# antonilo/unsupervised_detection

Measured on AMD Instinct MI355X. Metric: frame-pairs/sec per adversarial step, DAVIS 480p batch4, 1/2/4/8 GPU, higher is better.
Workload: dtype f32

## Files before the change

### include/udet_debug.h

```cpp
#ifndef UDET_DEBUG_H
#define UDET_DEBUG_H
#include <stddef.h>
#ifdef __cplusplus
extern "C" {
#endif
void udet_debug_force_conv(int bm, int bn, int ks);
void udet_debug_conv_fp16(int on);
void udet_debug_conv_fp16_grad_scale(float s);
void udet_debug_force_wgrad(int nsplit, int dma);
int udet_debug_last_wgrad(void);
int udet_debug_last_wgrad_reduce(void);
int udet_debug_conv2d_backward_filter_ex(const float* x, int ldx, int x_coff, const float* dy, int ldy, int y_coff, const float* y_saved, int act,
                                         float alpha, const float* w, const float* b, const float* gamma, float bn_c, float* dw, float* db,
                                         float* dgamma, float* dbeta, int n, int h, int wd, int cin, int cout, int k, int stride, int dilation,
                                         int up, void* workspace, size_t workspace_bytes, void* stream);
void udet_debug_upb_min_pixels(long v);
void udet_debug_set_tuning(int on);
void udet_debug_force_pair(int on);
int udet_debug_last_pair(void);
int udet_debug_conv2d_pair(const float* xa, const float* xb, const float* wa, const float* wb, const float* ba, const float* bb, float* ya, float* yb,
                           int na, int nb, int h, int w, int cin, int cout, int k, int stride, int dilation, int act, float alpha, void* workspace,
                           size_t workspace_bytes, void* stream);
#define UDET_DEBUG_UPCONV_WSETS_OFFSET 6400
size_t udet_debug_upconv_lowres_workspace_bytes(int ldx, int cin, int cout);
int udet_debug_upconv_lowres_fwd(const float* x, int ldx, const float* w, const float* bias, int act, float alpha, float* y, int ldy, int y_coff,
                                 float* xhat, int n, int h, int wd, int cin, int cout, int split, void* workspace, size_t workspace_bytes,
                                 void* stream);
int udet_debug_upconv_lowres_bwd(const float* dy, int ldy, int y_coff, const float* w, float* dx, int ldx, float* dxhat, int n, int h, int wd,
                                 int cin, int cout, void* workspace, size_t workspace_bytes, void* stream);
int udet_debug_upconv_tables(int h, int w, int backward, int* nseg, int* seg, int* seg_tap, int* taps, int taps_cap, int* ntaps);
int udet_debug_max_segs(void);
int udet_debug_last_conv(void);
#ifdef __cplusplus
}
#endif
#endif
```

### unsupervised_detection_amd/_devel.py

```python
from __future__ import annotations

import ctypes
import os

from ._ffi import check as _check, lib as _lib

_PATH = os.path.join(os.path.dirname(os.path.abspath(__file__)), "libudet_debug.so")
if not os.path.exists(_PATH):
    raise RuntimeError(f"{_PATH} is missing: build it with `make -C unsupervised_detection_amd/csrc`")
dbg = ctypes.CDLL(_PATH, mode=ctypes.RTLD_GLOBAL)
dbg.udet_debug_force_conv.restype = None
dbg.udet_debug_force_conv.argtypes = [ctypes.c_int, ctypes.c_int, ctypes.c_int]
dbg.udet_debug_last_conv.restype = ctypes.c_int
dbg.udet_debug_last_conv.argtypes = []
dbg.udet_debug_conv_fp16.restype = None
dbg.udet_debug_conv_fp16.argtypes = [ctypes.c_int]
dbg.udet_debug_conv_fp16_grad_scale.restype = None
dbg.udet_debug_conv_fp16_grad_scale.argtypes = [ctypes.c_float]
dbg.udet_debug_force_wgrad.restype = None
dbg.udet_debug_force_wgrad.argtypes = [ctypes.c_int, ctypes.c_int]
dbg.udet_debug_upb_min_pixels.restype = None
dbg.udet_debug_upb_min_pixels.argtypes = [ctypes.c_long]
dbg.udet_debug_set_tuning.restype = None
dbg.udet_debug_set_tuning.argtypes = [ctypes.c_int]
dbg.udet_debug_last_wgrad.restype = ctypes.c_int
dbg.udet_debug_last_wgrad.argtypes = []
dbg.udet_debug_force_pair.restype = None
dbg.udet_debug_force_pair.argtypes = [ctypes.c_int]
dbg.udet_debug_last_pair.restype = ctypes.c_int
dbg.udet_debug_last_pair.argtypes = []
dbg.udet_debug_conv2d_pair.restype = ctypes.c_int
dbg.udet_debug_conv2d_pair.argtypes = [ctypes.c_void_p] * 8 + [ctypes.c_int] * 10 + [ctypes.c_float, ctypes.c_void_p, ctypes.c_size_t, ctypes.c_void_p]
dbg.udet_debug_last_wgrad_reduce.restype = ctypes.c_int
dbg.udet_debug_last_wgrad_reduce.argtypes = []
_p, _i, _f = ctypes.c_void_p, ctypes.c_int, ctypes.c_float
dbg.udet_debug_conv2d_backward_filter_ex.restype = ctypes.c_int
dbg.udet_debug_conv2d_backward_filter_ex.argtypes = ([_p, _i, _i, _p, _i, _i, _p, _i, _f, _p, _p, _p, _f, _p, _p, _p, _p] + [_i] * 9
                                                     + [_p, ctypes.c_size_t, _p])
UPCONV_WSETS_OFFSET = 6400
dbg.udet_debug_upconv_lowres_workspace_bytes.restype = ctypes.c_size_t
dbg.udet_debug_upconv_lowres_workspace_bytes.argtypes = [_i, _i, _i]
dbg.udet_debug_upconv_lowres_fwd.restype = ctypes.c_int
dbg.udet_debug_upconv_lowres_fwd.argtypes = [_p, _i, _p, _p, _i, _f, _p, _i, _i, _p] + [_i] * 6 + [_p, ctypes.c_size_t, _p]
dbg.udet_debug_upconv_lowres_bwd.restype = ctypes.c_int
dbg.udet_debug_upconv_lowres_bwd.argtypes = [_p, _i, _i, _p, _p, _i, _p] + [_i] * 5 + [_p, ctypes.c_size_t, _p]
dbg.udet_debug_upconv_tables.restype = ctypes.c_int
dbg.udet_debug_upconv_tables.argtypes = [_i, _i, _i] + [_p] * 4 + [_i, _p]
dbg.udet_debug_max_segs.restype = ctypes.c_int
dbg.udet_debug_max_segs.argtypes = []


def upconv_tables(h: int, w: int, backward: bool):
    cap = 1024
    nseg, ntaps = ctypes.c_int(0), ctypes.c_int(0)
    seg, seg_tap, taps = (ctypes.c_int * 64)(), (ctypes.c_int * 17)(), (ctypes.c_int * (3 * cap))()
    st = dbg.udet_debug_upconv_tables(h, w, 1 if backward else 0, ctypes.addressof(nseg), ctypes.addressof(seg), ctypes.addressof(seg_tap),
                                      ctypes.addressof(taps), cap, ctypes.addressof(ntaps))
    _check(st)
    ns, nt = nseg.value, ntaps.value
    return dict(nseg=ns, seg=[tuple(seg[4 * s:4 * s + 4]) for s in range(ns)], seg_tap=list(seg_tap[:ns + 1]),
                taps=[tuple(taps[3 * t:3 * t + 3]) for t in range(nt)])
```

### unsupervised_detection_amd/csrc/conv_host.h

```cpp
#pragma once
#include "common.h"
namespace udet {
void same_pad(int in, int k, int s, int d, int* before, int* out);
void conv_setup_fwd(ConvParams& p, int N, int H, int W, int kh, int kw, int s, int d);
int conv_dgrad_classes(int s, int H, int W);
void conv_force_config(int bm, int bn, int ks);
bool conv_thin_n_ok(const ConvParams& p);
bool conv_thin_k_ok(const ConvParams& p);
int launch_conv_thin_n(const ConvParams& p, hipStream_t stream);
int launch_conv_thin_k(const ConvParams& p, hipStream_t stream);
bool conv_wino_geometry(const ConvParams& p, int* dil, int widx_at[9]);
bool conv_wino_ok(const ConvParams& p);
bool conv_wino_variant_ok(const ConvParams& p, int variant);
int conv_wino_np(int cout);
size_t conv_wino_floats(int Kc, int cout);
long conv_wino_workgroups(const ConvParams& p, int variant);
int conv_wino_max_ksplit(const ConvParams& p, int variant);
int launch_conv_wino(ConvParams& p, int variant, int ks, hipStream_t stream);
int launch_splitk_second_pass(const ConvParams& p, hipStream_t stream);
int launch_wino_pack(const float* src, float* dst, int R, int C, int Kc, int np, int k_split, int k_gap, int transposed, hipStream_t stream);
int launch_wino_from_packed(const ConvParams& p, float* dst, int np, hipStream_t stream);
void conv_debug_f16(int on);
int conv_debug_f16_on();
void conv_debug_f16_grad_scale(float s);
float conv_debug_f16_grad_scale_now();
int conv_last_config();
void conv_set_tuning(int on);
int tuned_shapes();
void tune_dump(FILE* f);
bool tune_put_line(const char* line);
int conv_tune_rejected();
void wgrad_set_tuning(int on);
bool wgrad_wino_ok(const WgradParams& p);
int wgrad_wino_slices(const WgradParams& p, int wanted);
int launch_wgrad_wino(const WgradParams& q, int slices, int ldn, hipStream_t stream);
int wgrad_last_config();
enum { WGRAD_RED_FUSED_BN = 1 << 26, WGRAD_RED_SEPARATE_BN = 1 << 27, WGRAD_RED_SWAPPED = 1 << 28, WGRAD_RED_CLASSES = 1 << 29 };
int wgrad_last_reduce();
void setup_up_fwd(ConvParams& p, int N, int H, int W);
void wgrad_force(int nsplit, int dma);
void conv_force_pair(int on);
int conv_last_pair();
#define UDET_TUNE_ABI 6
bool conv_setup_dgrad(ConvParams& p, int cls, int N, int H, int W, int kh, int kw, int s, int d);
int launch_pack_weights(const float* src, float* dst, int T, int R, int C, int Kc, int ldw, int k_split, int k_gap,
                        int mode, const float* scale, hipStream_t stream);
int launch_pack_taps_into_n(const float* src, float* dst, int T, int R, int C, int Kc, int ldz, int k_split, int k_gap,
                            int transposed, hipStream_t stream);
int launch_pack_jobs(const PackJob* jobs_dev, int njobs, const float* wsrc, float* ws, float bn_c, hipStream_t stream);
int launch_fold_bn(const float* b, const float* gamma, const float* beta, float c, float* scale, float* bias_f, int n,
                   hipStream_t stream);
int launch_copy_channels(const float* src, int lds, int s_coff, float* dst, int ldd, int d_coff, long P, int C, float mul,
                         float add, hipStream_t stream);
int launch_warp(const float* img, const float* flow, int ldf, int f_coff, float flow_scale, float* out, int N, int H,
                int W, int C, int* dbg_idx, float* dbg_alpha, hipStream_t stream);
int launch_cost_volume(const float* c1, const float* wr, float* out, int ldo, int o_coff, int N, int H, int W, int C,
                       hipStream_t stream);
int launch_warp_cost_volume(const float* c1, const float* c2, const float* flow, int ldf, int f_coff, float flow_scale, float* out,
                            int ldo, int corr_coff, int c1_coff, float* warped_dbg, int N, int H, int W, int C, hipStream_t stream);
inline int round_up(int v, int m) { return (v + m - 1) / m * m; }
}
```

### unsupervised_detection_amd/csrc/conv_wino.hip

```cpp
#include <string.h>

#include <mutex>
#include <type_traits>

#include "common.h"
#include "conv_epilogue.h"
#include "conv_host.h"
#include "wino_pack.h"

namespace udet {

typedef float floatx16 __attribute__((ext_vector_type(16)));

#ifdef UDET_EXPERIMENT
__device__ long long g_wino_ts[512 * 8];
#define WINO_STAMP(i)                                                                                  \
  do {                                                                                                 \
    if (threadIdx.x == 0 && blockIdx.x < 512 && blockIdx.z == 0) g_wino_ts[blockIdx.x * 8 + (i)] = (long long)__builtin_readcyclecounter(); \
  } while (0)
extern "C" int udet_exp_wino_stamps(long long* host, int n) {
  return (int)hipMemcpyFromSymbol(host, HIP_SYMBOL(g_wino_ts), (size_t)(n < 512 * 8 ? n : 512 * 8) * sizeof(long long));
}
#else
#define WINO_STAMP(i) do {} while (0)
#endif

static constexpr int wino_row_slots(int pw) { return (pw + 3) / 8 * 8 + 4; }

template <int WTY, int WTX, int WN>
struct WinoGeom {
  static constexpr int NS = 3;
  static constexpr int TH = 4 * WTY, TW = 8 * WTX;
  static constexpr int PH = 2 * TH + 2, PW = 2 * TW + 2;
  static constexpr int CS = PW / 2;
  static constexpr int S = wino_row_slots(PW);
  static constexpr int HP = S / 2;
  static constexpr int IN_SLOTS = 2 * PH * S;
  static constexpr int IN_INSTR = (IN_SLOTS + 255) / 256;
  static constexpr int IN_BYTES = IN_INSTR * 256 * 16;
  static constexpr int BN = 32 * WN;
  static constexpr int W_BYTES = 16 * 2 * BN * 16;
  static constexpr int W_INSTR = W_BYTES / 4096;
  static constexpr int STAGE = IN_BYTES + W_BYTES;
  static constexpr int L = IN_INSTR + W_INSTR;
  static constexpr int LA = (L + 1) / 2;
  static constexpr int LDS_BYTES = NS * STAGE;
  static_assert(S % 8 == 4 && S >= PW && HP >= CS, "row stride");
  static_assert(LDS_BYTES >= 4 * 128 * 32 * 4 && LDS_BYTES <= 160 * 1024, "the epilogue transposes 16 KB per wave through the stage buffers");
};

__device__ __forceinline__ float4 wino_bias_prefetch(const ConvParams& p, int n4) {
  return (p.ksplit <= 1 && (p.Cout & 3) == 0 && n4 < p.Cout) ? epi4_bias(p, n4) : make_float4(0.f, 0.f, 0.f, 0.f);
}
__device__ __forceinline__ void wino_store_block(const ConvParams& p, const float* xp, int lane, int n4, int n, int d, int sy, int sx, int Hs, int Ws,
                                                 int Yb, int Xb, const float4& bias_pre) {
  const bool slab = p.ksplit > 1;
  const bool vec = slab ? ((reinterpret_cast<uintptr_t>(p.partial) & 15) == 0 && (p.ldp & 3) == 0) : epilogue4_out_ok(p);
  const int c4 = (lane & 7) * 4;
  if (!slab && vec) {
    if (n4 >= p.Cout) return;
    const float4 bias = bias_pre;
    const EpiAct ea = epi_act(p);
    auto pix = [&](int P) {
      const int m = P >> 2, a = (P >> 1) & 1, b = P & 1;
      const int oy = Yb + 2 * (m >> 3) + a, ox = Xb + 2 * (m & 7) + b;
      return (oy >= Hs || ox >= Ws) ? -1 : (n * p.H + sy + d * oy) * p.W + sx + d * ox;
    };
    auto loop = [&](auto ELU) {
      if (epi4_plain(p)) {
#pragma unroll 1
        for (int k0 = 0; k0 < 16; k0 += 4) {
          float4 v[4];
          int off[4];
#pragma unroll
          for (int u = 0; u < 4; ++u) {
            const int P = (k0 + u) * 8 + (lane >> 3);
            v[u] = *reinterpret_cast<const float4*>(&xp[P * 32 + c4]);
            off[u] = pix(P);
          }
#pragma unroll
          for (int u = 0; u < 4; ++u)
            if (off[u] >= 0) epi4_finish_plain32<decltype(ELU)::value>(p, off[u], n4, v[u], bias, ea.slope);
        }
        return;
      }
#pragma unroll 1
      for (int k0 = 0; k0 < 16; k0 += 8) {
        float4 v[8];
        int off[8];
        Epi4Req rq[8];
#pragma unroll
        for (int u = 0; u < 8; ++u) {
          const int P = (k0 + u) * 8 + (lane >> 3);
          v[u] = *reinterpret_cast<const float4*>(&xp[P * 32 + c4]);
          off[u] = pix(P);
          if (off[u] >= 0) epi4_request(p, off[u], n4, rq[u]);
        }
#pragma unroll
        for (int u = 0; u < 8; ++u)
          if (off[u] >= 0) epi4_finish<decltype(ELU)::value>(p, off[u], n4, v[u], bias, rq[u], ea);
      }
    };
    if (p.act == ACT_ELU) loop(std::true_type());
// ... 290 lines not shown
      constexpr int RA[4] = {0, 1, 2, 1}, RB[4] = {2, 2, 1, 3};
      float vv[4][4];
#pragma unroll
      for (int j = 0; j < 4; ++j) {
        float t[4];
#pragma unroll
        for (int c = 0; c < 4; ++c) {
          const float a = comp(row[RA[i]][c], j), b = comp(row[RB[i]][c], j);
          t[c] = i == 1 ? a + b : a - b;
        }
        vv[j][0] = t[0] - t[2];
        vv[j][1] = t[1] + t[2];
        vv[j][2] = t[2] - t[1];
        vv[j][3] = t[1] - t[3];
      }
      __builtin_amdgcn_sched_barrier(0);
#pragma unroll
      for (int j = 0; j < 4; ++j)
#pragma unroll
        for (int q = 0; q < 4; ++q)
          acc[4 * i + q] = __builtin_amdgcn_mfma_f32_32x32x2f32(vv[j][q], comp(bfr[i & 1][q], j), acc[4 * i + q], 0, 0, 0);
      __builtin_amdgcn_sched_barrier(0);
      if (i == 2) {
        asm volatile("s_waitcnt vmcnt(0)" ::: "memory");
        __builtin_amdgcn_s_barrier();
        asm volatile("" ::: "memory");
      }
    }
    buf = b1;
  }

  __syncthreads();
  float* xp = reinterpret_cast<float*>(smem) + wave * (128 * 32);
#pragma unroll
  for (int r = 0; r < 16; ++r) {
    const int m = (r & 3) + 8 * (r >> 2) + 4 * lh;
    float s[4][2];
#pragma unroll
    for (int i = 0; i < 4; ++i) {
      s[i][0] = acc[i * 4 + 0][r] + acc[i * 4 + 1][r] + acc[i * 4 + 2][r];
      s[i][1] = acc[i * 4 + 1][r] - acc[i * 4 + 2][r] - acc[i * 4 + 3][r];
    }
#pragma unroll
    for (int b = 0; b < 2; ++b) {
      xp[(m * 4 + b) * 32 + li] = s[0][b] + s[1][b] + s[2][b];
      xp[(m * 4 + 2 + b) * 32 + li] = s[1][b] - s[2][b] - s[3][b];
    }
  }
  __builtin_amdgcn_wave_barrier();
  wino_store_block(p, xp, lane, nb * BN + wn * 32 + (lane & 7) * 4, n, d, sy, sx, Hs, Ws, Y0 + 8 * wty, X0 + 16 * wtx, bias_pre);
}

template <int WTY, int WTX, int WN>
__global__ __launch_bounds__(512) __attribute__((amdgpu_waves_per_eu(2, 2))) void conv_wino8_kernel(const ConvParams p, const int dil,
                                                                                                   const int BY, const int BX) {
  static_assert(WTY * WTX * WN == 4, "4 wave tiles");
  typedef WinoGeom<WTY, WTX, WN> G;
  constexpr int NS = G::NS, TH = G::TH, TW = G::TW, PH = G::PH, S = G::S, HP = G::HP, CS = G::CS;
  constexpr int IN_INSTR = G::IN_INSTR, IN_BYTES = G::IN_BYTES, BN = G::BN, STAGE = G::STAGE;
  constexpr int NW = G::W_BYTES / 1024;
  constexpr int PER = (IN_INSTR * 4 + NW + 7) / 8;
  constexpr int W0 = PER > IN_INSTR ? PER - IN_INSTR : 0;
  constexpr int W1 = (NW - 4 * W0) / 4;
  static_assert(W1 >= 0 && 4 * W0 + 4 * W1 == NW, "weight split");
  extern __shared__ __attribute__((aligned(16))) char smem[];
  WINO_STAMP(0);

  const int tid = threadIdx.x, lane = tid & 63, wave = __builtin_amdgcn_readfirstlane(tid >> 6);
  const int role = wave >> 2, sub = wave & 3;
  const int li = lane & 31, lh = lane >> 5;
  const int wn = sub % WN, wt = sub / WN, wty = wt / WTX, wtx = wt % WTX;

  int bid = xcd_tile_order(blockIdx.x, gridDim.x);
  const int NB = (p.Cout + BN - 1) / BN;
  const int nb = bid % NB;
  bid /= NB;
  const int d = dil;
  const int bx = bid % BX;
  int rem = bid / BX;
  const int by = rem % BY;
  rem /= BY;
  const int sx = rem % d;
  rem /= d;
  const int sy = rem % d;
  const int n = rem / d;
  const int Hs = (p.H - sy + d - 1) / d, Ws = (p.W - sx + d - 1) / d;
  const int Y0 = by * 2 * TH, X0 = bx * 2 * TW;
  const int nkg_all = p.Kc >> 3;
  int kg0 = 0, kg1 = nkg_all;
  if (p.ksplit > 1) {
    kg0 = (int)((long)nkg_all * blockIdx.z / p.ksplit);
    kg1 = (int)((long)nkg_all * (blockIdx.z + 1) / p.ksplit);
  }
  const int nkg = kg1 - kg0;

  unsigned in_voff[IN_INSTR];
  unsigned long long in_mask[IN_INSTR];
#pragma unroll
  for (int i = 0; i < IN_INSTR; ++i) {
    const int Lx = (i * 4 + sub) * 64 + lane;
    const int quad = Lx / (PH * S), r2 = Lx - quad * (PH * S);
    const int row = r2 / S, s = r2 - row * S;
    const int par = s / HP, cs = s - par * HP;
    const int col = 2 * cs + par;
    const int yy = Y0 - 1 + row, xx = X0 - 1 + col;
    const bool ok = quad < 2 && cs < CS && yy >= 0 && yy < Hs && xx >= 0 && xx < Ws;
    in_voff[i] = ok ? (unsigned)(((n * p.H + sy + d * yy) * p.W + sx + d * xx) * p.ldx + p.x_coff + quad * 4) * 4u : 0u;
    in_mask[i] = __ballot(ok);
    if (!ok && role == 0) {
#pragma unroll
      for (int b = 0; b < NS; ++b) *reinterpret_cast<float4*>(smem + b * STAGE + Lx * 16) = make_float4(0.f, 0.f, 0.f, 0.f);
    }
  }
  __syncthreads();
  WINO_STAMP(1);
  const int np = p.wino_np;
  const float4 bias_pre = wino_bias_prefetch(p, nb * BN + wn * 32 + (lane & 7) * 4);
  const float* ubase = p.wino_u + (size_t)nb * BN * 4;
  const size_t ustride = (size_t)32 * np * 4;
  const unsigned w_voff = BN == 32 ? (unsigned)((lane >> 5) * np + (lane & 31)) * 16 : (unsigned)lane * 16;
  const unsigned lds0 = (unsigned)(uintptr_t)(__attribute__((address_space(3))) char*)smem;
  auto dma_in = [&](int kg, int buf, int i) {
    asm volatile("s_mov_b32 m0, %2\n\ts_mov_b64 exec, %3\n\tglobal_load_lds_dwordx4 %0, %1\n\ts_mov_b64 exec, -1" ::"v"(in_voff[i]), "s"(p.x + kg * 8),
                 "s"(lds0 + buf * STAGE + (i * 4 + sub) * 1024), "s"(in_mask[i])
                 : "m0");
  };
  auto dma_w = [&](int kg, int buf, int w) {
    const float* us = ubase + (size_t)kg * ustride + (BN == 64 ? (size_t)w * np * 4 : (size_t)(2 * w) * np * 4);
    asm volatile("s_mov_b32 m0, %2\n\tglobal_load_lds_dwordx4 %0, %1" ::"v"(w_voff), "s"(us), "s"(lds0 + buf * STAGE + IN_BYTES + w * 1024) : "m0");
  };
  auto dma_part = [&](auto ROLE, int kg, int buf, int i0, int i1) {
    constexpr int R = decltype(ROLE)::value;
    constexpr int LR = R == 0 ? IN_INSTR + W0 : W1;
#pragma unroll
    for (int i = 0; i < LR; ++i) {
      if (i < i0 || i >= i1) continue;
      if (R == 0) {
        if (i < IN_INSTR) dma_in(kg, buf, i);
        else dma_w(kg, buf, (i - IN_INSTR) * 4 + sub);
      } else {
        dma_w(kg, buf, 4 * W0 + i * 4 + sub);
      }
    }
  };

  floatx16 acc[8];
#pragma unroll
  for (int q = 0; q < 8; ++q)
#pragma unroll
    for (int r = 0; r < 16; ++r) acc[q][r] = 0.f;

  const int ty = li >> 3, tx = li & 7;
  const int a_base = ((lh * PH + 2 * (wty * 4 + ty)) * S + (wtx * 8 + tx)) * 16;
  const int b_base = IN_BYTES + (lh * BN + wn * 32 + li) * 16;
  auto ld_row = [&](const char* sb, int r, float4 (&dst)[4]) {
#pragma unroll
    for (int c = 0; c < 4; ++c) dst[c] = *reinterpret_cast<const float4*>(sb + a_base + (r * S + (c & 1) * HP + (c >> 1)) * 16);
  };
  auto ld_bf = [&](const char* sb, int i, float4 (&dst)[4]) {
#pragma unroll
    for (int q = 0; q < 4; ++q) dst[q] = *reinterpret_cast<const float4*>(sb + b_base + (4 * i + q) * (2 * BN * 16));
  };
  auto comp = [](const float4& v, int j) { return j == 0 ? v.x : (j == 1 ? v.y : (j == 2 ? v.z : v.w)); };

  auto body = [&](auto ROLE) {
    constexpr int R = decltype(ROLE)::value;
    constexpr int LR = R == 0 ? IN_INSTR + W0 : W1;
    constexpr int LA = (LR + 1) / 2;
    constexpr int I0 = R == 0 ? 1 : 0, I1 = R == 0 ? 2 : 3;
    float4 ra[4], rb[4];
    float4 rc[4], rd[4];
    float4 bf0[4], bf1[4];
    float v1[4][4];
#pragma unroll
    for (int c = 0; c < 4; ++c) ra[c] = rb[c] = rc[c] = rd[c] = bf0[c] = bf1[c] = make_float4(0.f, 0.f, 0.f, 0.f);
    if (nkg > 0) dma_part(ROLE, kg0, 0, 0, LR);
    if (nkg > 1) dma_part(ROLE, kg0 + 1, 1, 0, LR);
    if (nkg > 1) asm volatile("s_waitcnt vmcnt(%0)" ::"n"(LR) : "memory");
    else asm volatile("s_waitcnt vmcnt(0)" ::: "memory");
    __builtin_amdgcn_s_barrier();
    asm volatile("" ::: "memory");
    WINO_STAMP(2);
    ld_row(smem, R == 0 ? 1 : 0, ra);
    ld_row(smem, 2, rb);
    ld_bf(smem, I0, bf0);
    int buf = 0;
    for (int k = 0; k < nkg; ++k) {
      const char* sb = smem + buf * STAGE;
      const int b1 = buf + 1 == NS ? 0 : buf + 1, b2 = b1 + 1 == NS ? 0 : b1 + 1;
      const char* sbn = smem + b1 * STAGE;
      if (R == 1) { ld_row(sb, 1, rc); ld_row(sb, 3, rd); }
      ld_bf(sb, I1, bf1);
      if (k > 0 && k + 1 < nkg) dma_part(ROLE, kg0 + k + 1, b1, LA, LR);
      __builtin_amdgcn_sched_barrier(0);
#pragma unroll
      for (int j = 0; j < 4; ++j) {
        float t[4], v[4];
#pragma unroll
        for (int c = 0; c < 4; ++c) {
          const float a = comp(ra[c], j), b = comp(rb[c], j);
          t[c] = R == 0 ? a + b : a - b;
        }
        v[0] = t[0] - t[2]; v[1] = t[1] + t[2]; v[2] = t[2] - t[1]; v[3] = t[1] - t[3];
        if (R == 0) {
          float u[4];
#pragma unroll
          for (int c = 0; c < 4; ++c) u[c] = comp(rb[c], j) - comp(ra[c], j);
          v1[j][0] = u[0] - u[2]; v1[j][1] = u[1] + u[2]; v1[j][2] = u[2] - u[1]; v1[j][3] = u[1] - u[3];
        }
#pragma unroll
        for (int q = 0; q < 4; ++q) acc[q] = __builtin_amdgcn_mfma_f32_32x32x2f32(v[q], comp(bf0[q], j), acc[q], 0, 0, 0);
      }
      __builtin_amdgcn_sched_barrier(0);
      asm volatile("s_waitcnt vmcnt(0)" ::: "memory");
      __builtin_amdgcn_s_barrier();
      asm volatile("" ::: "memory");
      ld_row(sbn, R == 0 ? 1 : 0, ra);
      ld_row(sbn, 2, rb);
      ld_bf(sbn, I0, bf0);
      if (k + 2 < nkg) dma_part(ROLE, kg0 + k + 2, b2, 0, LA);
      __builtin_amdgcn_sched_barrier(0);
#pragma unroll
      for (int j = 0; j < 4; ++j) {
        float v[4];
        if (R == 0) {
#pragma unroll
          for (int q = 0; q < 4; ++q) v[q] = v1[j][q];
        } else {
          float t[4];
#pragma unroll
          for (int c = 0; c < 4; ++c) t[c] = comp(rc[c], j) - comp(rd[c], j);
          v[0] = t[0] - t[2]; v[1] = t[1] + t[2]; v[2] = t[2] - t[1]; v[3] = t[1] - t[3];
        }
#pragma unroll
        for (int q = 0; q < 4; ++q) acc[4 + q] = __builtin_amdgcn_mfma_f32_32x32x2f32(v[q], comp(bf1[q], j), acc[4 + q], 0, 0, 0);
      }
      __builtin_amdgcn_sched_barrier(0);
      buf = b1;
    }
  };
  if (role == 0) body(std::integral_constant<int, 0>());
  else body(std::integral_constant<int, 1>());

  WINO_STAMP(3);
  __syncthreads();
  wino_roles_epilogue(p, acc, reinterpret_cast<float*>(smem) + sub * 4096, role, lane, nb * BN + wn * 32 + (lane & 7) * 4, n, d, sy, sx, Hs, Ws, Y0 + 8 * wty,
                      X0 + 16 * wtx, bias_pre);
#ifdef UDET_EXPERIMENT
  WINO_STAMP(5);
  asm volatile("s_waitcnt vmcnt(0)" ::: "memory");
  WINO_STAMP(6);
#endif
}

struct WinoHalfGeom {
  static constexpr int NS = 2, TH = 4, TW = 8;
  static constexpr int PH = 2 * TH + 2, PW = 2 * TW + 2;
  static constexpr int CS = PW / 2, S = wino_row_slots(PW), HP = S / 2;
  static constexpr int IN_SLOTS = 2 * PH * S;
  static constexpr int IN_WINSTR = (IN_SLOTS + 63) / 64;
  static constexpr int IN_INSTR = (IN_WINSTR + 3) / 4;
  static constexpr int IN_BYTES = IN_WINSTR * 1024;
  static constexpr int BN = 64;
  static constexpr int W_BYTES = 16 * 2 * BN * 16;
  static constexpr int NW = W_BYTES / 1024;
  static constexpr int STAGE = IN_BYTES + W_BYTES;
  static constexpr int LDS_BYTES = NS * STAGE;
  static_assert(LDS_BYTES >= 4 * 128 * 32 * 4 && 2 * LDS_BYTES <= 160 * 1024, "epilogue scratch / two workgroups per CU");
};
__global__ __launch_bounds__(256) __attribute__((amdgpu_waves_per_eu(2, 2))) void conv_wino_half_kernel(const ConvParams p, const int dil, const int BY,
                                                                                                       const int BX) {
  typedef WinoHalfGeom G;
  constexpr int TH = G::TH, TW = G::TW, PH = G::PH, S = G::S, HP = G::HP, CS = G::CS;
  constexpr int IN_INSTR = G::IN_INSTR, IN_BYTES = G::IN_BYTES, BN = G::BN, STAGE = G::STAGE, NW = G::NW;
  extern __shared__ __attribute__((aligned(16))) char smem[];

  const int tid = threadIdx.x, lane = tid & 63, wave = __builtin_amdgcn_readfirstlane(tid >> 6);
  const int role = wave >> 1, wn = wave & 1;
  const int li = lane & 31, lh = lane >> 5;

  int bid = xcd_tile_order(blockIdx.x, gridDim.x);
  const int NB = (p.Cout + BN - 1) / BN;
  const int nb = bid % NB;
  bid /= NB;
  const int d = dil;
  const int bx = bid % BX;
  int rem = bid / BX;
  const int by = rem % BY;
  rem /= BY;
  const int sx = rem % d;
  rem /= d;
  const int sy = rem % d;
  const int n = rem / d;
  const int Hs = (p.H - sy + d - 1) / d, Ws = (p.W - sx + d - 1) / d;
  const int Y0 = by * 2 * TH, X0 = bx * 2 * TW;
  const int nkg_all = p.Kc >> 3;
  int kg0 = 0, kg1 = nkg_all;
  if (p.ksplit > 1) {
// ... 162 lines not shown
      for (int a = 0; a < 3; ++a)
#pragma unroll
        for (int b = 0; b < 3; ++b) val += Gm[pi][a] * Gm[pj][b] * wp[((long)tm.w[a * 3 + b] * Kc + k) * ldw + n];
    }
    dst[e] = val;
  }
}
int launch_wino_from_packed(const ConvParams& p, float* dst, int np, hipStream_t stream) {
  int d = 0;
  WinoTapMap tm;
  if (!conv_wino_geometry(p, &d, tm.w)) {
    set_error("wino: the launch is not a 3x3 stride-1 convolution");
    return UDET_ERR_UNSUPPORTED;
  }
  const long total = (long)(p.Kc / 8) * 16 * 2 * np * 4;
  int nb = (int)((total + 255) / 256);
  if (nb > 2048) nb = 2048;
  UDET_LAUNCH(wino_from_packed_kernel, dim3(nb), dim3(256), 0, stream, p.wp, p.Kc, p.ldw, tm, dst, np, total);
  UDET_HIP(hipGetLastError());
  return UDET_OK;
}

int conv_wino_np(int cout) { return cout > 64 ? round_up(cout, 128) : (cout > 32 ? 64 : 32); }
size_t conv_wino_floats(int Kc, int cout) { return (size_t)(Kc / 8) * 16 * 2 * conv_wino_np(cout) * 4; }

bool conv_wino_geometry(const ConvParams& p, int* dil, int widx_at[9]) {
  if (p.ntaps != 9 || p.ncls == 4 || p.up_shift != 0) return false;
  if (p.isy != 1 || p.isx != 1 || p.osy != 1 || p.osx != 1 || p.ooy != 0 || p.oox != 0) return false;
  if (p.OH != p.H || p.OW != p.W || p.OHq != p.OH || p.OWq != p.OW) return false;
  int d = 0;
  for (int t = 0; t < 9; ++t) {
    const int a = p.taps[t].dy < 0 ? -p.taps[t].dy : p.taps[t].dy;
    if (a > d) d = a;
  }
  if (d < 1) return false;
  for (int i = 0; i < 9; ++i) widx_at[i] = -1;
  for (int t = 0; t < 9; ++t) {
    const int dy = p.taps[t].dy, dx = p.taps[t].dx;
    if (dy % d != 0 || dx % d != 0) return false;
    const int a = dy / d + 1, b = dx / d + 1;
    if (a < 0 || a > 2 || b < 0 || b > 2 || widx_at[a * 3 + b] >= 0) return false;
    widx_at[a * 3 + b] = p.taps[t].widx;
  }
  *dil = d;
  return true;
}
bool conv_wino_ok(const ConvParams& p) {
  if (p.nseg) return false;
  int d, w[9];
  if (p.f16 || p.xa != nullptr || p.wino_u == nullptr || p.zero16 == nullptr) return false;
  if ((reinterpret_cast<uintptr_t>(p.zero16) | reinterpret_cast<uintptr_t>(p.wino_u) | reinterpret_cast<uintptr_t>(p.x)) & 15) return false;
  if (p.Kc < 8 || p.Kc % 8 != 0 || p.ldx % 4 != 0 || p.x_coff % 4 != 0) return false;
  if (p.wino_np < 32 || p.wino_np % 32 != 0 || p.wino_np < p.Cout) return false;
  if ((long)p.N * p.H * p.W * (long)p.ldy >= (1L << 31) || (long)p.N * p.H * p.W * (long)p.ldx >= (1L << 30)) return false;
  return conv_wino_geometry(p, &d, w);
}
static int variant_bn(int v) { return v == 4 ? 64 : ((v & 1) == 0 ? 64 : 32); }
bool conv_wino_variant_ok(const ConvParams& p, int v) {
  if (v < 0 || v > 4) return false;
  const int bn = variant_bn(v);
  if (p.wino_np % bn != 0) return false;
  return p.Cout > bn / 2 || bn == 32;
}
static void variant_blocks(const ConvParams& p, int v, int d, int* BY, int* BX) {
  const int th = v == 4 ? 4 : 8, tw = (v & 1) ? 16 : 8;
  const int Hs = (p.H + d - 1) / d, Ws = (p.W + d - 1) / d;
  *BY = (Hs + 2 * th - 1) / (2 * th);
  *BX = (Ws + 2 * tw - 1) / (2 * tw);
}
long conv_wino_workgroups(const ConvParams& p, int v) {
  int d, w[9], BY, BX;
  if (!conv_wino_geometry(p, &d, w)) return 0;
  variant_blocks(p, v, d, &BY, &BX);
  return (long)p.N * d * d * BY * BX * ((p.Cout + variant_bn(v) - 1) / variant_bn(v));
}
int conv_wino_max_ksplit(const ConvParams& p, int v) {
  (void)v;
  if (!p.partial) return 1;
  int ks = (p.Kc / 8) / 6;
  if (ks > 16) ks = 16;
  const size_t per_split = (size_t)p.N * p.H * p.W * ((p.Cout + 3) & ~3);
  while (ks > 1 && per_split * ks > p.partial_cap) --ks;
  return ks < 1 ? 1 : ks;
}
int launch_splitk_second_pass(const ConvParams& p, hipStream_t stream);

template <int WTY, int WTX, int WN, bool EIGHT>
static int launch_variant(const ConvParams& p, int d, int BY, int BX, hipStream_t stream) {
  typedef WinoGeom<WTY, WTX, WN> G;
  auto kern = EIGHT ? conv_wino8_kernel<WTY, WTX, WN> : conv_wino_kernel<WTY, WTX, WN>;
  static std::once_flag once;
  static hipError_t attr = hipSuccess;
  std::call_once(once, [&]() { attr = hipFuncSetAttribute(reinterpret_cast<const void*>(kern), hipFuncAttributeMaxDynamicSharedMemorySize, G::LDS_BYTES); });
  UDET_HIP(attr);
  dim3 grid(p.N * d * d * BY * BX * ((p.Cout + G::BN - 1) / G::BN), 1, p.ksplit > 1 ? p.ksplit : 1);
  UDET_LAUNCH(kern, grid, dim3(EIGHT ? 512 : 256), G::LDS_BYTES, stream, p, d, BY, BX);
  UDET_HIP(hipGetLastError());
  return UDET_OK;
}
static int launch_half(const ConvParams& p, int d, int BY, int BX, hipStream_t stream) {
  typedef WinoHalfGeom G;
  static std::once_flag once;
  static hipError_t attr = hipSuccess;
  std::call_once(once, [&]() { attr = hipFuncSetAttribute(reinterpret_cast<const void*>(conv_wino_half_kernel), hipFuncAttributeMaxDynamicSharedMemorySize, G::LDS_BYTES); });
  UDET_HIP(attr);
  dim3 grid(p.N * d * d * BY * BX * ((p.Cout + G::BN - 1) / G::BN), 1, p.ksplit > 1 ? p.ksplit : 1);
  UDET_LAUNCH(conv_wino_half_kernel, grid, dim3(256), G::LDS_BYTES, stream, p, d, BY, BX);
  UDET_HIP(hipGetLastError());
  return UDET_OK;
}
int launch_conv_wino(ConvParams& p, int variant, int ks, hipStream_t stream) {
  int d, w[9], BY, BX;
  if (!conv_wino_ok(p) || !conv_wino_geometry(p, &d, w) || !conv_wino_variant_ok(p, variant)) {
    set_error("wino: launch not eligible (variant %d)", variant);
    return UDET_ERR_UNSUPPORTED;
  }
  variant_blocks(p, variant, d, &BY, &BX);
  const int cap = conv_wino_max_ksplit(p, variant);
  p.ksplit = ks > cap ? cap : (ks < 1 ? 1 : ks);
  p.fold = 0; p.tail_full = 0; p.tail_ks = 0; p.tail_prow0 = 0;
  p.ncls = 1;
  if (p.ksplit > 1) p.ldp = (p.Cout + 3) & ~3;
  int rc;
  if (variant == 0) rc = launch_variant<2, 1, 2, false>(p, d, BY, BX, stream);
  else if (variant == 1) rc = launch_variant<2, 2, 1, false>(p, d, BY, BX, stream);
  else if (variant == 2) rc = launch_variant<2, 1, 2, true>(p, d, BY, BX, stream);
  else if (variant == 4) rc = launch_half(p, d, BY, BX, stream);
  else rc = launch_variant<2, 2, 1, true>(p, d, BY, BX, stream);
  if (rc != UDET_OK) return rc;
  if (p.ksplit > 1) return launch_splitk_second_pass(p, stream);
  return UDET_OK;
}

}
```

### unsupervised_detection_amd/csrc/devel/api_debug.hip

```cpp
#include <string.h>

#include <vector>

#include "../../../include/udet_debug.h"
#include "../conv_host.h"
#include "../plan_run.h"

using namespace udet;

extern "C" {
int udet_debug_last_conv(void) { return conv_last_config(); }
void udet_debug_force_conv(int bm, int bn, int ks) { conv_force_config(bm, bn, ks); }
void udet_debug_conv_fp16(int on) { conv_debug_f16(on); }
void udet_debug_conv_fp16_grad_scale(float s) { conv_debug_f16_grad_scale(s); }
void udet_debug_force_wgrad(int nsplit, int dma) { wgrad_force(nsplit, dma); }
int udet_debug_last_wgrad(void) { return wgrad_last_config(); }
int udet_debug_last_wgrad_reduce(void) { return wgrad_last_reduce(); }
int udet_debug_conv2d_backward_filter_ex(const float* x, int ldx, int x_coff, const float* dy, int ldy, int y_coff, const float* y_saved, int act,
                                         float alpha, const float* w, const float* b, const float* gamma, float bn_c, float* dw, float* db,
                                         float* dgamma, float* dbeta, int n, int h, int wd, int cin, int cout, int k, int stride, int dilation,
                                         int up, void* workspace, size_t workspace_bytes, void* stream_) {
  hipStream_t stream = (hipStream_t)stream_;
  if (!x || !dy || !dw || n < 1 || h < 1 || wd < 1 || cin < 1 || cout < 1 || k < 1 || k * k > UDET_MAX_TAPS || dilation < 1 ||
      (stride != 1 && stride != 2) || up < 0 || up > 2) {
    set_error("debug_backward_filter_ex: bad argument");
    return UDET_ERR_ARG;
  }
  if (ldx % 4 || x_coff % 4 || ldy % 4 || y_coff % 4) {
    set_error("debug_backward_filter_ex: ldx=%d x_coff=%d ldy=%d y_coff=%d must be multiples of 4", ldx, x_coff, ldy, y_coff);
    return UDET_ERR_ALIGN;
  }
  if (x_coff < 0 || y_coff < 0 || x_coff + round_up(cin, 4) > ldx || y_coff + round_up(cout, 4) > ldy) {
    set_error("debug_backward_filter_ex: channel window outside the buffer (x %d+%d of %d, dy %d+%d of %d)", x_coff, cin, ldx, y_coff, cout, ldy);
    return UDET_ERR_SHAPE;
  }
  if (gamma && (!w || !b || !db || !dgamma || !dbeta)) {
    set_error("debug_backward_filter_ex: a BN-folded layer needs w, b, db, dgamma and dbeta");
    return UDET_ERR_ARG;
  }
  if (up == 2 && (!gamma || y_saved || k != 3 || stride != 1 || dilation != 1)) {
    set_error("debug_backward_filter_ex: the class-structured form is a BN-folded 3x3 stride-1 layer on dU");
    return UDET_ERR_ARG;
  }
  if (!workspace || (reinterpret_cast<uintptr_t>(workspace) & 63) || workspace_bytes < 128 * sizeof(float)) {
    set_error("debug_backward_filter_ex: workspace must be 64-byte aligned and hold the zero block");
    return UDET_ERR_ARG;
  }
  float* zero = reinterpret_cast<float*>(workspace);
  const int us = up ? 1 : 0;
  WgradParams p;
  memset(&p, 0, sizeof(p));
  p.x = x; p.ldx = ldx; p.x_coff = x_coff; p.N = n; p.Cin = cin;
  p.dy = dy; p.ldy = ldy; p.y_coff = y_coff; p.Cout = cout;
  if (y_saved && act != UDET_ACT_NONE) { p.ya = y_saved; p.yact = act; p.yalpha = alpha; }
  p.dw = dw; p.db = db;
  p.partial = zero + 64; p.partial_floats = workspace_bytes / sizeof(float) - 64;
  p.zero16 = zero;
  p.f16_yscale = conv_debug_f16_grad_scale_now();
  if (gamma) { p.w = w; p.b = b; p.gamma = gamma; p.dgamma = dgamma; p.dbeta = dbeta; p.bn_c = bn_c; }
  ConvParams g;
  memset(&g, 0, sizeof(g));
  conv_setup_fwd(g, n, h << us, wd << us, k, k, stride, dilation);
  p.H = h << us; p.W = wd << us; p.up_shift = us;
  p.OH = g.OH; p.OW = g.OW; p.isy = p.isx = stride;
  p.ntaps = g.ntaps;
  memcpy(p.taps, g.taps, sizeof(g.taps));
  UDET_HIP(hipMemsetAsync(zero, 0, 64 * sizeof(float), stream));
  if (up == 2) return launch_wgrad_up_T(p, h, wd, stream);
  return launch_wgrad_T(p, k * k, stream);
}
void udet_debug_upb_min_pixels(long v) { plan_debug_upb_min_pixels(v); }
void udet_debug_force_pair(int on) { conv_force_pair(on); }
int udet_debug_last_pair(void) { return conv_last_pair(); }
int udet_debug_conv2d_pair(const float* xa, const float* xb, const float* wa, const float* wb, const float* ba, const float* bb, float* ya, float* yb,
                           int na, int nb, int h, int w, int cin, int cout, int k, int stride, int dilation, int act, float alpha, void* workspace,
                           size_t workspace_bytes, void* stream_) {
  hipStream_t stream = (hipStream_t)stream_;
  if (cin % 8 != 0 || k * k > UDET_MAX_TAPS) { set_error("debug_conv2d_pair: cin must be a multiple of 8"); return UDET_ERR_SHAPE; }
  const int kc = cin, ldw = round_up(cout, 4);
  const size_t wfl = ((size_t)k * k * kc * ldw + 63) & ~(size_t)63, part_fl = (size_t)4 << 20, zero_fl = 64 + UDET_MAX_TICKETS;
  if (workspace_bytes < (2 * wfl + part_fl + zero_fl) * sizeof(float)) { set_error("debug_conv2d_pair: workspace too small"); return UDET_ERR_ARG; }
  float* wpa = reinterpret_cast<float*>(workspace);
  float* wpb = wpa + wfl;
  float* part = wpb + wfl;
  float* zero = part + part_fl;
  UDET_HIP(hipMemsetAsync(zero, 0, zero_fl * sizeof(float), stream));
  UDET_TRY(launch_pack_weights(wa, wpa, k * k, cin, cout, kc, ldw, kc, 0, 0, nullptr, stream));
  UDET_TRY(launch_pack_weights(wb, wpb, k * k, cin, cout, kc, ldw, kc, 0, 0, nullptr, stream));
  ConvParams p[2];
  for (int i = 0; i < 2; ++i) {
    memset(&p[i], 0, sizeof(ConvParams));
    conv_setup_fwd(p[i], i ? nb : na, h, w, k, k, stride, dilation);
    p[i].x = i ? xb : xa; p[i].ldx = cin; p[i].wp = i ? wpb : wpa; p[i].Kc = kc; p[i].ldw = ldw; p[i].bias = i ? bb : ba;
    p[i].y = i ? yb : ya; p[i].ldy = cout; p[i].Cout = cout; p[i].act = act; p[i].alpha = alpha;
    p[i].partial = part; p[i].partial_cap = part_fl; p[i].zero16 = zero; p[i].tickets = reinterpret_cast<int*>(zero + 64);
  }
  return launch_conv_pair(p[0], p[1], stream);
}
}
namespace {
enum { UPC_TICKETS = 64, UPC_JOBS = UPC_TICKETS + UDET_MAX_TICKETS, UPC_JOBS_CAP = 192, UPC_TAB = UPC_JOBS + UPC_JOBS_CAP, UPC_TAB_CAP = 2048,
       UPC_WSETS = UPC_TAB + UPC_TAB_CAP, UPC_MIN_SLAB = 1 << 20 };
static_assert(UPC_WSETS == UDET_DEBUG_UPCONV_WSETS_OFFSET && UPC_WSETS % 64 == 0 && 8 * sizeof(PackJob) <= UPC_JOBS_CAP * sizeof(float), "workspace layout");
size_t upc_align64(size_t v) { return (v + 63) & ~(size_t)63; }
int upc_kct(int cout) { return round_up(cout, cout <= 4 ? 4 : 8); }
size_t upc_floats(int kc, int ldw) { return UPC_WSETS + upc_align64((size_t)4 * 36 * kc * ldw) + UPC_MIN_SLAB; }
int upc_check(const char* who, const void* a, const void* b, const void* c, const void* d, int n, int h, int wd, int cin, int cout, void* workspace,
              size_t workspace_bytes, size_t need_floats) {
  if (!a || !b || !c || !d || n < 1 || cin < 1 || cout < 1) { set_error("%s: bad argument", who); return UDET_ERR_ARG; }
  if (h < 2 || wd < 2) { set_error("%s: the source grid %d x %d must be at least 2 x 2 (one interior row / column and the last one)", who, h, wd); return UDET_ERR_SHAPE; }
  if ((long)n * (2 * h) * (2 * wd) >= (1L << 28)) { set_error("%s: grid too large", who); return UDET_ERR_SHAPE; }
  if (!workspace || (reinterpret_cast<uintptr_t>(workspace) & 63) || workspace_bytes < need_floats * sizeof(float)) {
    set_error("%s: workspace must be 64-byte aligned and hold %zu bytes", who, need_floats * sizeof(float));
    return UDET_ERR_ARG;
  }
  return UDET_OK;
}
int upc_stage(const Layer::SegLaunch& tab, const std::vector<PackJob>& jobs, const float* w, float* ws, hipStream_t stream) {
  if (tab.taps.size() * sizeof(ConvTap) > UPC_TAB_CAP * sizeof(float) || jobs.size() * sizeof(PackJob) > UPC_JOBS_CAP * sizeof(float)) {
    set_error("debug_upconv_lowres: table larger than its workspace slot");
    return UDET_ERR_ARG;
  }
  UDET_HIP(hipMemsetAsync(ws, 0, UPC_JOBS * sizeof(float), stream));
  UDET_HIP(hipMemcpyAsync(ws + UPC_JOBS, jobs.data(), jobs.size() * sizeof(PackJob), hipMemcpyHostToDevice, stream));
// ... 127 lines not shown
```

Baseline: 501.1.

## Pass compact Winograd-8 kernel header, defer full ConvParams load until after first DMA

The 8-wave Winograd kernel now takes a small packed header (pointers plus bit-packed dims) as leading kernel arguments and reads the large ConvParams struct from the kernarg segment only after the first input/weight DMAs are issued. This is meant to cut the prologue latency of loading a large kernarg struct into scalar registers before useful memory traffic starts. It adds dimension-range guards for the 16-bit packing and relies on manual kernarg offset arithmetic, which is fragile if the struct layout or alignment changes. It also adds debug entry points for testing the header and windowed convs.

```diff
diff --git a/include/udet_debug.h b/include/udet_debug.h
--- a/include/udet_debug.h
+++ b/include/udet_debug.h
@@ -16,6 +16,10 @@
                                          int up, void* workspace, size_t workspace_bytes, void* stream);
 void udet_debug_upb_min_pixels(long v);
 void udet_debug_set_tuning(int on);
+int udet_debug_wino_head(const float* x, const float* u, const float* bias, int H, int W, int ldx, int x_coff, int Kc, int np, int cout, int ksplit,
+                         int dil, int by, int bx, int nwg, long long* out);
+int udet_debug_conv2d_window(const float* x, int ldx, int x_coff, const float* w, const float* bias, float* y, int ldy, int y_coff, int n, int h, int wd,
+                             int cin, int cout, int k, int dilation, int act, float alpha, void* workspace, size_t workspace_bytes, void* stream);
 void udet_debug_force_pair(int on);
 int udet_debug_last_pair(void);
 int udet_debug_conv2d_pair(const float* xa, const float* xb, const float* wa, const float* wb, const float* ba, const float* bb, float* ya, float* yb,
diff --git a/unsupervised_detection_amd/_devel.py b/unsupervised_detection_amd/_devel.py
--- a/unsupervised_detection_amd/_devel.py
+++ b/unsupervised_detection_amd/_devel.py
@@ -25,6 +25,11 @@
 dbg.udet_debug_set_tuning.argtypes = [ctypes.c_int]
 dbg.udet_debug_last_wgrad.restype = ctypes.c_int
 dbg.udet_debug_last_wgrad.argtypes = []
+dbg.udet_debug_wino_head.restype = ctypes.c_int
+dbg.udet_debug_wino_head.argtypes = [ctypes.c_void_p] * 3 + [ctypes.c_int] * 12 + [ctypes.POINTER(ctypes.c_longlong)]
+dbg.udet_debug_conv2d_window.restype = ctypes.c_int
+dbg.udet_debug_conv2d_window.argtypes = ([ctypes.c_void_p, ctypes.c_int, ctypes.c_int, ctypes.c_void_p, ctypes.c_void_p, ctypes.c_void_p] + [ctypes.c_int] * 10 +
+                                         [ctypes.c_float, ctypes.c_void_p, ctypes.c_size_t, ctypes.c_void_p])
 dbg.udet_debug_force_pair.restype = None
 dbg.udet_debug_force_pair.argtypes = [ctypes.c_int]
 dbg.udet_debug_last_pair.restype = ctypes.c_int
diff --git a/unsupervised_detection_amd/csrc/conv_host.h b/unsupervised_detection_amd/csrc/conv_host.h
--- a/unsupervised_detection_amd/csrc/conv_host.h
+++ b/unsupervised_detection_amd/csrc/conv_host.h
@@ -17,6 +17,17 @@
 long conv_wino_workgroups(const ConvParams& p, int variant);
 int conv_wino_max_ksplit(const ConvParams& p, int variant);
 int launch_conv_wino(ConvParams& p, int variant, int ks, hipStream_t stream);
+struct WinoHead {
+  const float *x, *u, *bias;
+  int hw;
+  int ldx, x_coff;
+  int kcnp;
+  int Cout;
+  int nwg;
+  int byx;
+  int dks;
+};
+WinoHead wino_head(const ConvParams& p, int d, int BY, int BX, int nwg);
 int launch_splitk_second_pass(const ConvParams& p, hipStream_t stream);
 int launch_wino_pack(const float* src, float* dst, int R, int C, int Kc, int np, int k_split, int k_gap, int transposed, hipStream_t stream);
 int launch_wino_from_packed(const ConvParams& p, float* dst, int np, hipStream_t stream);
diff --git a/unsupervised_detection_amd/csrc/conv_wino.hip b/unsupervised_detection_amd/csrc/conv_wino.hip
--- a/unsupervised_detection_amd/csrc/conv_wino.hip
+++ b/unsupervised_detection_amd/csrc/conv_wino.hip
@@ -49,6 +49,11 @@
   static_assert(LDS_BYTES >= 4 * 128 * 32 * 4 && LDS_BYTES <= 160 * 1024, "the epilogue transposes 16 KB per wave through the stage buffers");
 };
 
+__device__ __forceinline__ void wino_late_params(ConvParams& q, const ConvParams& p) {
+  constexpr size_t A1 = offsetof(ConvParams, ntaps), B0 = offsetof(ConvParams, zero16);
+  __builtin_memcpy(&q, &p, A1);
+  __builtin_memcpy(reinterpret_cast<char*>(&q) + B0, reinterpret_cast<const char*>(&p) + B0, sizeof(ConvParams) - B0);
+}
 __device__ __forceinline__ float4 wino_bias_prefetch(const ConvParams& p, int n4) {
   return (p.ksplit <= 1 && (p.Cout & 3) == 0 && n4 < p.Cout) ? epi4_bias(p, n4) : make_float4(0.f, 0.f, 0.f, 0.f);
 }
@@ -445,8 +450,9 @@
 }
 
 template <int WTY, int WTX, int WN>
-__global__ __launch_bounds__(512) __attribute__((amdgpu_waves_per_eu(2, 2))) void conv_wino8_kernel(const ConvParams p, const int dil,
-                                                                                                   const int BY, const int BX) {
+__global__ __launch_bounds__(512) __attribute__((amdgpu_waves_per_eu(2, 2))) void conv_wino8_kernel(
+    const float* __restrict__ h_x, const float* __restrict__ h_u, const float* __restrict__ h_bias, const int h_hw, const int h_ldx, const int h_xcoff,
+    const int h_kcnp, const int h_Cout, const int h_nwg, const int h_byx, const int h_dks, const ConvParams p_late) {
   static_assert(WTY * WTX * WN == 4, "4 wave tiles");
   typedef WinoGeom<WTY, WTX, WN> G;
   constexpr int NS = G::NS, TH = G::TH, TW = G::TW, PH = G::PH, S = G::S, HP = G::HP, CS = G::CS;
@@ -458,14 +464,21 @@
   static_assert(W1 >= 0 && 4 * W0 + 4 * W1 == NW, "weight split");
   extern __shared__ __attribute__((aligned(16))) char smem[];
   WINO_STAMP(0);
+  typedef const __attribute__((address_space(4))) char* KargPtr;
+  constexpr int P_OFF = ((int)sizeof(WinoHead) + (int)alignof(ConvParams) - 1) / (int)alignof(ConvParams) * (int)alignof(ConvParams);
+  KargPtr kp = (KargPtr)__builtin_amdgcn_kernarg_segment_ptr() + P_OFF;
+  (void)p_late;
+  ConvParams q;
 
   const int tid = threadIdx.x, lane = tid & 63, wave = __builtin_amdgcn_readfirstlane(tid >> 6);
   const int role = wave >> 2, sub = wave & 3;
   const int li = lane & 31, lh = lane >> 5;
   const int wn = sub % WN, wt = sub / WN, wty = wt / WTX, wtx = wt % WTX;
 
-  int bid = xcd_tile_order(blockIdx.x, gridDim.x);
-  const int NB = (p.Cout + BN - 1) / BN;
+  const int dil = h_dks & 255, h_ksplit = h_dks >> 8, BY = h_byx & 65535, BX = h_byx >> 16;
+  const int h_H = h_hw & 65535, h_W = h_hw >> 16, h_Kc = h_kcnp & 65535, h_np = h_kcnp >> 16;
+  int bid = xcd_tile_order(blockIdx.x, h_nwg);
+  const int NB = (h_Cout + BN - 1) / BN;
   const int nb = bid % NB;
   bid /= NB;
   const int d = dil;
@@ -477,13 +490,13 @@
   rem /= d;
   const int sy = rem % d;
   const int n = rem / d;
-  const int Hs = (p.H - sy + d - 1) / d, Ws = (p.W - sx + d - 1) / d;
+  const int Hs = (h_H - sy + d - 1) / d, Ws = (h_W - sx + d - 1) / d;
   const int Y0 = by * 2 * TH, X0 = bx * 2 * TW;
-  const int nkg_all = p.Kc >> 3;
+  const int nkg_all = h_Kc >> 3;
   int kg0 = 0, kg1 = nkg_all;
-  if (p.ksplit > 1) {
-    kg0 = (int)((long)nkg_all * blockIdx.z / p.ksplit);
-    kg1 = (int)((long)nkg_all * (blockIdx.z + 1) / p.ksplit);
+  if (h_ksplit > 1) {
+    kg0 = (int)((long)nkg_all * blockIdx.z / h_ksplit);
+    kg1 = (int)((long)nkg_all * (blockIdx.z + 1) / h_ksplit);
   }
   const int nkg = kg1 - kg0;
 
@@ -498,7 +511,7 @@
     const int col = 2 * cs + par;
     const int yy = Y0 - 1 + row, xx = X0 - 1 + col;
     const bool ok = quad < 2 && cs < CS && yy >= 0 && yy < Hs && xx >= 0 && xx < Ws;
-    in_voff[i] = ok ? (unsigned)(((n * p.H + sy + d * yy) * p.W + sx + d * xx) * p.ldx + p.x_coff + quad * 4) * 4u : 0u;
+    in_voff[i] = ok ? (unsigned)(((n * h_H + sy + d * yy) * h_W + sx + d * xx) * h_ldx + h_xcoff + quad * 4) * 4u : 0u;
     in_mask[i] = __ballot(ok);
     if (!ok && role == 0) {
 #pragma unroll
@@ -507,14 +520,17 @@
   }
   __syncthreads();
   WINO_STAMP(1);
-  const int np = p.wino_np;
-  const float4 bias_pre = wino_bias_prefetch(p, nb * BN + wn * 32 + (lane & 7) * 4);
-  const float* ubase = p.wino_u + (size_t)nb * BN * 4;
+  const int np = h_np;
+  const int n4_pre = nb * BN + wn * 32 + (lane & 7) * 4;
+  const float4 bias_pre = (h_ksplit <= 1 && (h_Cout & 3) == 0 && n4_pre < h_Cout && h_bias)
+                              ? make_float4(h_bias[n4_pre], h_bias[n4_pre + 1], h_bias[n4_pre + 2], h_bias[n4_pre + 3])
+                              : make_float4(0.f, 0.f, 0.f, 0.f);
+  const float* ubase = h_u + (size_t)nb * BN * 4;
   const size_t ustride = (size_t)32 * np * 4;
   const unsigned w_voff = BN == 32 ? (unsigned)((lane >> 5) * np + (lane & 31)) * 16 : (unsigned)lane * 16;
   const unsigned lds0 = (unsigned)(uintptr_t)(__attribute__((address_space(3))) char*)smem;
   auto dma_in = [&](int kg, int buf, int i) {
-    asm volatile("s_mov_b32 m0, %2\n\ts_mov_b64 exec, %3\n\tglobal_load_lds_dwordx4 %0, %1\n\ts_mov_b64 exec, -1" ::"v"(in_voff[i]), "s"(p.x + kg * 8),
+    asm volatile("s_mov_b32 m0, %2\n\ts_mov_b64 exec, %3\n\tglobal_load_lds_dwordx4 %0, %1\n\ts_mov_b64 exec, -1" ::"v"(in_voff[i]), "s"(h_x + kg * 8),
                  "s"(lds0 + buf * STAGE + (i * 4 + sub) * 1024), "s"(in_mask[i])
                  : "m0");
   };
@@ -569,6 +585,8 @@
     for (int c = 0; c < 4; ++c) ra[c] = rb[c] = rc[c] = rd[c] = bf0[c] = bf1[c] = make_float4(0.f, 0.f, 0.f, 0.f);
     if (nkg > 0) dma_part(ROLE, kg0, 0, 0, LR);
     if (nkg > 1) dma_part(ROLE, kg0 + 1, 1, 0, LR);
+    asm volatile("" : "+s"(kp));
+    wino_late_params(q, *(const ConvParams*)(const __attribute__((address_space(4))) ConvParams*)kp);
     if (nkg > 1) asm volatile("s_waitcnt vmcnt(%0)" ::"n"(LR) : "memory");
     else asm volatile("s_waitcnt vmcnt(0)" ::: "memory");
     __builtin_amdgcn_s_barrier();
@@ -637,6 +655,7 @@
 
   WINO_STAMP(3);
   __syncthreads();
+  const ConvParams& p = q;
   wino_roles_epilogue(p, acc, reinterpret_cast<float*>(smem) + sub * 4096, role, lane, nb * BN + wn * 32 + (lane & 7) * 4, n, d, sy, sx, Hs, Ws, Y0 + 8 * wty,
                       X0 + 16 * wtx, bias_pre);
 #ifdef UDET_EXPERIMENT
@@ -905,8 +924,20 @@
   if ((reinterpret_cast<uintptr_t>(p.zero16) | reinterpret_cast<uintptr_t>(p.wino_u) | reinterpret_cast<uintptr_t>(p.x)) & 15) return false;
   if (p.Kc < 8 || p.Kc % 8 != 0 || p.ldx % 4 != 0 || p.x_coff % 4 != 0) return false;
   if (p.wino_np < 32 || p.wino_np % 32 != 0 || p.wino_np < p.Cout) return false;
+  if (p.H >= 32768 || p.W >= 32768 || p.Kc >= 32768 || p.wino_np >= 32768) return false;
   if ((long)p.N * p.H * p.W * (long)p.ldy >= (1L << 31) || (long)p.N * p.H * p.W * (long)p.ldx >= (1L << 30)) return false;
   return conv_wino_geometry(p, &d, w);
+}
+WinoHead wino_head(const ConvParams& p, int d, int BY, int BX, int nwg) {
+  WinoHead h;
+  h.x = p.x; h.u = p.wino_u; h.bias = p.bias;
+  h.hw = p.H | (p.W << 16);
+  h.ldx = p.ldx; h.x_coff = p.x_coff;
+  h.kcnp = p.Kc | (p.wino_np << 16);
+  h.Cout = p.Cout; h.nwg = nwg;
+  h.byx = BY | (BX << 16);
+  h.dks = d | ((p.ksplit > 1 ? p.ksplit : 1) << 8);
+  return h;
 }
 static int variant_bn(int v) { return v == 4 ? 64 : ((v & 1) == 0 ? 64 : 32); }
 bool conv_wino_variant_ok(const ConvParams& p, int v) {
@@ -941,13 +972,21 @@
 template <int WTY, int WTX, int WN, bool EIGHT>
 static int launch_variant(const ConvParams& p, int d, int BY, int BX, hipStream_t stream) {
   typedef WinoGeom<WTY, WTX, WN> G;
-  auto kern = EIGHT ? conv_wino8_kernel<WTY, WTX, WN> : conv_wino_kernel<WTY, WTX, WN>;
+  auto kern = [] {
+    if constexpr (EIGHT) return conv_wino8_kernel<WTY, WTX, WN>;
+    else return conv_wino_kernel<WTY, WTX, WN>;
+  }();
   static std::once_flag once;
   static hipError_t attr = hipSuccess;
   std::call_once(once, [&]() { attr = hipFuncSetAttribute(reinterpret_cast<const void*>(kern), hipFuncAttributeMaxDynamicSharedMemorySize, G::LDS_BYTES); });
   UDET_HIP(attr);
   dim3 grid(p.N * d * d * BY * BX * ((p.Cout + G::BN - 1) / G::BN), 1, p.ksplit > 1 ? p.ksplit : 1);
-  UDET_LAUNCH(kern, grid, dim3(EIGHT ? 512 : 256), G::LDS_BYTES, stream, p, d, BY, BX);
+  if constexpr (EIGHT) {
+    const WinoHead h = wino_head(p, d, BY, BX, (int)grid.x);
+    UDET_LAUNCH(kern, grid, dim3(512), G::LDS_BYTES, stream, h.x, h.u, h.bias, h.hw, h.ldx, h.x_coff, h.kcnp, h.Cout, h.nwg, h.byx, h.dks, p);
+  } else {
+    UDET_LAUNCH(kern, grid, dim3(256), G::LDS_BYTES, stream, p, d, BY, BX);
+  }
   UDET_HIP(hipGetLastError());
   return UDET_OK;
 }
diff --git a/unsupervised_detection_amd/csrc/devel/api_debug.hip b/unsupervised_detection_amd/csrc/devel/api_debug.hip
--- a/unsupervised_detection_amd/csrc/devel/api_debug.hip
+++ b/unsupervised_detection_amd/csrc/devel/api_debug.hip
@@ -70,6 +70,40 @@
   return launch_wgrad_T(p, k * k, stream);
 }
 void udet_debug_upb_min_pixels(long v) { plan_debug_upb_min_pixels(v); }
+int udet_debug_wino_head(const float* x, const float* u, const float* bias, int H, int W, int ldx, int x_coff, int Kc, int np, int cout, int ksplit,
+                         int dil, int by, int bx, int nwg, long long* out) {
+  ConvParams p;
+  memset(&p, 0, sizeof(p));
+  p.x = x; p.wino_u = u; p.bias = bias; p.H = H; p.W = W; p.ldx = ldx; p.x_coff = x_coff; p.Kc = Kc; p.wino_np = np; p.Cout = cout; p.ksplit = ksplit;
+  const WinoHead h = wino_head(p, dil, by, bx, nwg);
+  out[0] = (long long)(uintptr_t)h.x; out[1] = (long long)(uintptr_t)h.u; out[2] = (long long)(uintptr_t)h.bias;
+  out[3] = h.hw; out[4] = h.ldx; out[5] = h.x_coff; out[6] = h.kcnp; out[7] = h.Cout; out[8] = h.nwg; out[9] = h.byx; out[10] = h.dks;
+  return (int)sizeof(WinoHead);
+}
+int udet_debug_conv2d_window(const float* x, int ldx, int x_coff, const float* w, const float* bias, float* y, int ldy, int y_coff, int n, int h, int wd,
+                             int cin, int cout, int k, int dilation, int act, float alpha, void* workspace, size_t workspace_bytes, void* stream_) {
+  hipStream_t stream = (hipStream_t)stream_;
+  if (cin % 8 != 0 || k * k > UDET_MAX_TAPS || ldx % 4 || x_coff % 4 || x_coff < 0 || x_coff + cin > ldx || y_coff < 0 || y_coff + cout > ldy || n < 1 ||
+      h < 1 || wd < 1 || cout < 1 || dilation < 1) {
+    set_error("debug_conv2d_window: bad window (x %d+%d of %d, y %d+%d of %d)", x_coff, cin, ldx, y_coff, cout, ldy);
+    return UDET_ERR_SHAPE;
+  }
+  const int kc = cin, ldw = round_up(cout, 4);
+  const size_t wfl = ((size_t)k * k * kc * ldw + 63) & ~(size_t)63, part_fl = (size_t)4 << 20, zero_fl = 64 + UDET_MAX_TICKETS;
+  if (workspace_bytes < (wfl + part_fl + zero_fl) * sizeof(float)) { set_error("debug_conv2d_window: workspace too small"); return UDET_ERR_ARG; }
+  float* wp = reinterpret_cast<float*>(workspace);
+  float* part = wp + wfl;
+  float* zero = part + part_fl;
+  UDET_HIP(hipMemsetAsync(zero, 0, zero_fl * sizeof(float), stream));
+  UDET_TRY(launch_pack_weights(w, wp, k * k, cin, cout, kc, ldw, kc, 0, 0, nullptr, stream));
+  ConvParams p;
+  memset(&p, 0, sizeof(p));
+  conv_setup_fwd(p, n, h, wd, k, k, 1, dilation);
+  p.x = x; p.ldx = ldx; p.x_coff = x_coff; p.wp = wp; p.Kc = kc; p.ldw = ldw; p.bias = bias;
+  p.y = y; p.ldy = ldy; p.y_coff = y_coff; p.Cout = cout; p.act = act; p.alpha = alpha;
+  p.partial = part; p.partial_cap = part_fl; p.zero16 = zero; p.tickets = reinterpret_cast<int*>(zero + 64);
+  return launch_conv(p, stream);
+}
 void udet_debug_force_pair(int on) { conv_force_pair(on); }
 int udet_debug_last_pair(void) { return conv_last_pair(); }
 int udet_debug_conv2d_pair(const float* xa, const float* xb, const float* wa, const float* wb, const float* ba, const float* bb, float* ya, float* yb,
```

After: 501.7, median of 6. About the same (+0.1%).
